# EricPedley/ORB_SLAM3_ROS2

Measured on AMD Instinct MI355X. Metric: frames/sec ORB extract+match @640×480; KF/sec LocalBA (50 KF, 2k pts), higher is better.
Workload: dtype u8; 1 GPU; C2: 640x480, 8-level pyramid, 1000 feat/frame, FAST 20/7, batch=1 per camera stream; ORBextractor::operator() + brute-force Hamming match to the camera's previous frame; step=one frame on each of 16 independent camera streams, parallelism=replicas x1 (no collective); 16 camera streams per GPU, batch 1 each, cameras=16

## Files before the change

### orb_slam3_ros2_amd/csrc/extract.cpp

```cpp
#include "extract.h"

#include <algorithm>
#include <cstdlib>
#include <cstring>
#include <map>
#include <memory>
#include <mutex>
#include <vector>

#include "devbuf.h"
#include "graph_cache.h"
#include "orbhip_kernels.h"
#include "stage.h"

#define HIPOK(x) ORBHIP_HIPOK(" extract", x)

namespace orbhip {
namespace {

struct Plan {
    HostPlan hp;
    DevBuf<ExtractPlan> d_plan;
    DevBuf<CellGeom> d_cells;
    DevBuf<int> d_xofs, d_xalpha, d_yofs, d_ybeta, d_disc, d_cone_tab, d_cone_hi_tab, d_bands, d_flow_dep;
// ... 139 lines not shown
    HIPOK(ws->grow(ws->d_pyr, (size_t)B * P.pyr_bytes));
    HIPOK(ws->grow(ws->d_cand, (size_t)B * P.n_slots_total));
    HIPOK(ws->grow(ws->d_cprim, (size_t)B * P.n_cells_total * kCandPrim));
    HIPOK(ws->grow(ws->d_kscratch, (size_t)B * P.n_slots_total));
    HIPOK(ws->grow(ws->d_nscratch, (size_t)B * P.n_slots_total));
    HIPOK(ws->grow(ws->d_cand_cnt, (size_t)B * P.n_cells_total));
    HIPOK(ws->grow(ws->d_cand_off, (size_t)B * P.n_cells_total));
    HIPOK(ws->grow(ws->d_cand_fill, (size_t)B * kMaxLevels));
    if (pl->hp.flow_nbt) {
        const uint64_t was = ws->gen;
        HIPOK(ws->grow(ws->d_flow, kFlowCtl + (size_t)B * pl->hp.flow_nbt));
        if (ws->gen != was) HIPOK(hipMemset(ws->d_flow.p, 0, ws->d_flow.n * sizeof(int)));
    }
    HIPOK(ws->grow(ws->d_lvl_kp, (size_t)B * P.kp_slots_total));
    HIPOK(ws->grow(ws->d_lvl_cnt, (size_t)B * P.n_levels));
    HIPOK(ws->grow(ws->d_lvl_nlap, (size_t)B * P.n_levels));
    HIPOK(ws->grow(ws->d_err, 4));
    return ORBHIP_OK;
}

static void launch_pyramid(ExtractWorkspace* ws, Plan* pl, FrameBufs& fb, int B, const RunSwitches& sw, bool flow_on,
                           hipStream_t st) {
    const ExtractPlan& P = pl->hp.h;
    StageTimer& tm = *ws->timer;
    static const size_t cone_max = std::getenv("ORBHIP_CONE_MAX_WG")
                                       ? (size_t)std::atol(std::getenv("ORBHIP_CONE_MAX_WG"))
                                       : (size_t)1024;
    const bool cone_path = pl->hp.cone_tiles && !sw.no_cone && (size_t)B * pl->hp.cone_tiles <= cone_max;
    const bool cone_hi = !cone_path && pl->hp.cone_hi_tiles && sw.cone_hi;
    fb.stamp = (cone_path && tm.stage == 1 && tm.dstamp && tm.n < StageTimer::kCap) ? tm.dstamp + tm.n : nullptr;
    if (cone_path) {
        static const int cone_nt = [] {
            const char* e = std::getenv("ORBHIP_CONE_NT");
            const int v = e ? std::atoi(e) : 1024;
            return (v == 256 || v == 512) ? v : 1024;
        }();
        launch_pyr_cone(pl->d_plan.p, pl->hp.cone_tiles, pl->hp.cone_lds, fb, B, pl->d_cone.p, pl->d_cone_tab.p,
                        pl->hp.cone_tab_stride, st, 0, cone_nt, pl->d_xofs.p, pl->d_xalpha.p, pl->d_yofs.p,
                        pl->d_ybeta.p);
    } else if (flow_on) {
        PyrFlow fa{};
        fa.ctl = ws->d_flow.p;
        fa.flags = ws->d_flow.p + kFlowCtl;
        fa.dep = (const int2*)pl->d_flow_dep.p;
        for (int l = 0; l <= kMaxLevels; l++) fa.boff[l] = pl->hp.flow_boff[l];
        fa.B = B;
        fa.nbt = pl->hp.flow_nbt;
        fa.pyr_limit = (int)((int64_t)B * P.pyr_bytes);
        launch_pyr_flow(pl->d_plan.p, fb, pl->d_xofs.p, pl->d_xalpha.p, pl->d_yofs.p, pl->d_ybeta.p, fa, st);
    } else {
        const bool bands = !cone_hi && pl->hp.nbands > 0;
        const int lr = cone_hi ? kConeHiStart + 1 : (bands ? kBandStart + 1 : P.n_levels);
        for (int l = 1; l < lr; l++)
            launch_resize(pl->d_plan.p, P, fb, B, l, pl->d_xofs.p, pl->d_xalpha.p, pl->d_yofs.p, pl->d_ybeta.p,
                          st);
        if (cone_hi)
            launch_pyr_cone(pl->d_plan.p, pl->hp.cone_hi_tiles, pl->hp.cone_hi_lds, fb, B, pl->d_cone_hi.p,
                            pl->d_cone_hi_tab.p, pl->hp.cone_hi_tab_stride, st, kConeHiStart, cone_hi_threads(),
                            pl->d_xofs.p, pl->d_xalpha.p, pl->d_yofs.p, pl->d_ybeta.p);
        if (bands)
            launch_resize_bands(pl->d_plan.p, pl->hp.nbands, fb, B, kBandStart, (const int2*)pl->d_bands.p,
                                pl->d_xofs.p, pl->d_xalpha.p, pl->d_yofs.p, pl->d_ybeta.p, st);
    }
}

static int run_extract(ExtractWorkspace* ws, Plan* pl, const uint8_t* d_imgs, int B, int stride, int64_t fstride,
                       int lap0, int lap1, orbhip_kp* d_kps, uint8_t* d_desc, int cap, int32_t* d_n, int32_t* d_mono,
                       hipStream_t st) {
    const ExtractPlan& P = pl->hp.h;
    (void)hipGetLastError();
    int rc = ensure_batch(ws, pl, B);
    if (rc) return rc;
    const RunSwitches sw = read_run_switches();
    const bool flow_on = sw.flow && pl->hp.flow_nbt > 0 && (int64_t)B * P.pyr_bytes < (1ll << 31);
    GraphKey key;
    key.add(1).add((uint64_t)sw.oct_fast).add((uint64_t)sw.oct_max_dh).add((uint64_t)sw.no_cone)
        .add((uint64_t)sw.cone_hi).add((uint64_t)flow_on).add((uint64_t)sw.pack).add((uint64_t)ws->fast_nt).ptr(pl)
        .ptr(d_imgs).add((uint64_t)B).add((uint64_t)stride).add((uint64_t)fstride).add((uint64_t)lap0)
        .add((uint64_t)lap1).ptr(d_kps).ptr(d_desc).add((uint64_t)cap).ptr(d_n).ptr(d_mono).ptr(st)
        .ptr(ws).add(ws->gen);
    return ws->graphs->run(key, st, ws->timer->stage != 0, [&](hipStream_t st) -> int {
        FrameBufs fb;
        fb.in = d_imgs; fb.in_stride = stride; fb.in_fstride = fstride; fb.pyr = ws->d_pyr.p;
        StageTimer& tm = *ws->timer;
        const StageScope scope(tm);
        tm.begin(1, st);
        launch_pyramid(ws, pl, fb, B, sw, flow_on, st);
        tm.end(1, st);
        tm.begin(2, st);
        CandPack cp;
        cp.prim = ws->d_cprim.p;
        if (sw.pack) {
// ... 191 lines not shown
```

### orb_slam3_ros2_amd/csrc/extract_kernels.hip

```cpp
#include <hip/hip_runtime.h>
#include <cstdlib>
#include <type_traits>

#include "../../include/orbhip.h"
#include "dev_attr.h"
#include "../../include/orbhip_pattern.h"
#include "orbhip_device.h"
#include "orbhip_kernels.h"
#include "orbhip_plan.h"

namespace orbhip {

__constant__ __attribute__((visibility("hidden"))) signed char kPattern[256 * 4] = ORBHIP_BIT_PATTERN_31_INIT;

ORBHIP_TRACE_UNIT(extract)

struct ImgRef {
    const uint8_t* p;
    int pitch;
};

__device__ __forceinline__ ImgRef level_img(const ExtractPlan* __restrict__ P, const FrameBufs& fb, int f, int l) {
    if (l == 0) return ImgRef{fb.in + (int64_t)f * fb.in_fstride, fb.in_stride};
    return ImgRef{fb.pyr + (int64_t)f * P->pyr_bytes + P->lv[l].pyr_off, P->lv[l].pitch};
// ... 279 lines not shown
                        typedef unsigned int u32x4v __attribute__((ext_vector_type(4)));
                        const u32x4v u = {v.x, v.y, v.z, v.w};
                        __builtin_amdgcn_raw_buffer_store_b128(u, prs, obase + (dyb + r) * pitch + c, 0, 16);
                    }
                    wave_lds_only();
                }
            }
            asm volatile("s_waitcnt vmcnt(0)" ::: "memory");
            __syncthreads();
            if (tid == 0)
                __hip_atomic_store((ex_gint*)(fl + a.boff[l] + b), gen + 1, __ATOMIC_RELAXED,
                                   __HIP_MEMORY_SCOPE_AGENT);
            if (tr_k < 32) { TR_PHASE(7, 2 * tr_k + 1) }
            tr_k++;
        }
    }
    TR_END(7)
    if (tid == 0 && atomicAdd(ctl + kFlowQ, 1) == (int)gridDim.x - 1) {
        for (int i = 0; i <= kFlowQ; i++)
            __hip_atomic_store((ex_gint*)(ctl + i), 0, __ATOMIC_RELAXED, __HIP_MEMORY_SCOPE_AGENT);
        __hip_atomic_store((ex_gint*)(ctl + kFlowQ + 1), gen + 1, __ATOMIC_RELAXED, __HIP_MEMORY_SCOPE_AGENT);
    }
}

__device__ __forceinline__ int small_div(int i, float inv_d) { return (int)(((float)i + 0.5f) * inv_d); }

__device__ __forceinline__ void wait_vm_all() { asm volatile("s_waitcnt vmcnt(0)" ::: "memory"); }
__device__ __forceinline__ void lds_only_barrier() {
    asm volatile("s_waitcnt lgkmcnt(0)" ::: "memory");
    __builtin_amdgcn_s_barrier();
    asm volatile("" ::: "memory");
}

__device__ __forceinline__ void pyr_cone_body(const ExtractPlan* __restrict__ P, const FrameBufs& fb,
                                              const ConeRect* __restrict__ rects, const int* __restrict__ ctab,
                                              int tab_stride, uint8_t* __restrict__ cone, int tile, int f, int s0) {
    TR_BEGIN()
    const int L = P->n_levels, tid = threadIdx.x, nt = blockDim.x;
    const ConeRect* R = rects + (size_t)tile * kMaxLevels;
    static_assert(sizeof(ConeRect) == 16 && kMaxLevels * 4 <= 64 && (kMaxLevels & (kMaxLevels - 1)) == 0, "4 dwords per level");
    const uint32_t rdw = ((const uint32_t*)R)[threadIdx.x & (4 * kMaxLevels - 1)];
    auto rect = [&](int l) -> ConeRect {
        const uint32_t d0 = (uint32_t)__builtin_amdgcn_readlane((int)rdw, 4 * l),
                       d1 = (uint32_t)__builtin_amdgcn_readlane((int)rdw, 4 * l + 1),
                       d2 = (uint32_t)__builtin_amdgcn_readlane((int)rdw, 4 * l + 2),
                       d3 = (uint32_t)__builtin_amdgcn_readlane((int)rdw, 4 * l + 3);
        return ConeRect{(int16_t)(d0 & 0xFFFF), (int16_t)(d0 >> 16), (int16_t)(d1 & 0xFFFF), (int16_t)(d1 >> 16),
                        (int16_t)(d2 & 0xFFFF), (int16_t)(d2 >> 16), (int16_t)(d3 & 0xFFFF), (int16_t)(d3 >> 16)};
    };
    int boff[kMaxLevels], toff[kMaxLevels];
    int tot = 0;
    const ConeRect Rs0 = rect(s0);
    const int P0 = (Rs0.nx1 - Rs0.nx0 + 6) & ~3;
    for (int l = s0; l < L; l++) {
        const ConeRect r = rect(l);
        boff[l] = tot;
        tot += ((l == s0 ? P0 : (r.nx1 - r.nx0)) * (r.ny1 - r.ny0) + 15) & ~15;
    }
    int sh0 = 0;
    int* tab = (int*)(cone + tot);
    int ttot = 0;
    for (int l = s0 + 1; l < L; l++) {
        toff[l] = ttot;
        const ConeRect r = rect(l);
        ttot += 2 * (r.nx1 - r.nx0) + 3 * (r.ny1 - r.ny0);
    }
    const int* gt = ctab + (size_t)tile * tab_stride;
    auto tab_at = [&](int i) -> int { return gt[i]; };
    TR_PHASE(0, 20)
    {
        const ImgRef in0 = level_img(P, fb, f, s0);
        const ConeRect r = Rs0;
        const int nw = r.nx1 - r.nx0, nh = r.ny1 - r.ny0;
        const uint8_t* src0 = in0.p + (int64_t)r.ny0 * in0.pitch + r.nx0;
        const bool dw = ((in0.pitch & 3) == 0) && ((((uintptr_t)in0.p) & 3) == 0);
        if (dw) sh0 = (int)(((uintptr_t)src0) & 3);
        const int nwd = dw ? (nw + sh0 + 3) >> 2 : 0;
        const int tot0 = dw ? nwd * nh : nw * nh;
        const float inv_n = 1.0f / (float)(dw ? nwd : nw);
        uint8_t* lv0 = cone + boff[s0];
        if (dw && tot0 <= 1024 && ttot <= 2 * 1024 && nt == 1024) {
            const uint32_t* s4 = (const uint32_t*)(src0 - sh0);
            const int p4 = in0.pitch >> 2;
            int tv[2];
#pragma unroll
            for (int u = 0; u < 2; u++) tv[u] = gt[min(tid + 1024 * u, ttot - 1)];
            const int i = min(tid, tot0 - 1);
            const int y = small_div(i, inv_n), x = i - y * nwd;
            const uint32_t v = s4[(int64_t)y * p4 + x];
#pragma unroll
            for (int u = 0; u < 2; u++)
                if (tid + 1024 * u < ttot) tab[tid + 1024 * u] = tv[u];
            if (tid < tot0) ((uint32_t*)lv0)[y * (P0 >> 2) + x] = v;
            TR_PHASE(0, 21)
        } else if (dw) {
            const uint32_t* s4 = (const uint32_t*)(src0 - sh0);
            const int p4 = in0.pitch >> 2;
            constexpr int U = 8;
            for (int i0 = tid; i0 < ttot; i0 += U * nt) {
                int v[U];
#pragma unroll
                for (int u = 0; u < U; u++) v[u] = tab_at(min(i0 + u * nt, ttot - 1));
#pragma unroll
                for (int u = 0; u < U; u++)
                    if (i0 + u * nt < ttot) tab[i0 + u * nt] = v[u];
            }
            for (int i0 = tid; i0 < tot0; i0 += U * nt) {
                uint32_t v[U];
                int o[U];
#pragma unroll
                for (int u = 0; u < U; u++) {
                    const int i = min(i0 + u * nt, tot0 - 1);
                    const int y = small_div(i, inv_n), x = i - y * nwd;
                    v[u] = s4[(int64_t)y * p4 + x];
                    o[u] = y * (P0 >> 2) + x;
                }
#pragma unroll
                for (int u = 0; u < U; u++)
                    if (i0 + u * nt < tot0) ((uint32_t*)lv0)[o[u]] = v[u];
            }
        } else {
            for (int i = tid; i < ttot; i += nt) tab[i] = tab_at(i);
            for (int i = tid; i < tot0; i += nt) {
                const int y = small_div(i, inv_n), x = i - y * nw;
                lv0[y * P0 + x] = src0[(int64_t)y * in0.pitch + x];
            }
        }
    }
    __syncthreads();
    TR_PHASE(0, 0)
    for (int l = s0 + 1; l < L; l++) {
        const LevelGeom& D = P->lv[l];
        const ConeRect r = rect(l), rp = rect(l - 1);
        const int nw = r.nx1 - r.nx0, nh = r.ny1 - r.ny0, nwp = l == s0 + 1 ? P0 : rp.nx1 - rp.nx0;
        const int* t = tab + toff[l];
        const uint8_t* src = cone + boff[l - 1] + (l == s0 + 1 ? sh0 : 0);
        uint8_t* dst = fb.pyr + (int64_t)f * P->pyr_bytes + D.pyr_off;
        const float inv_nw = 1.0f / (float)nw;
        const bool noclamp = D.rz_noclamp != 0;
        for (int i = tid; i < nw * nh; i += nt) {
            const int yy = small_div(i, inv_nw), xx = i - yy * nw;
            const int x = r.nx0 + xx, y = r.ny0 + yy;
            const int sx = t[xx] - rp.nx0;
            const uint8_t* S0 = src + (t[2 * nw + 3 * yy] - rp.ny0) * nwp;
            const uint8_t* S1 = src + (t[2 * nw + 3 * yy + 1] - rp.ny0) * nwp;
            int h0, h1;
            if (x < D.xmax) {
                const int aa = t[nw + xx];
                const int a0 = (int)(short)(aa & 0xFFFF), a1 = (int)(short)(aa >> 16);
                h0 = S0[sx] * a0 + S0[sx + 1] * a1;
                h1 = S1[sx] * a0 + S1[sx + 1] * a1;
            } else {
                h0 = S0[sx] * 2048;
                h1 = S1[sx] * 2048;
            }
            const int bb = t[2 * nw + 3 * yy + 2];
            const int b0 = (int)(short)(bb & 0xFFFF), b1 = (int)(short)(bb >> 16);
            int v;
            if (x < D.vend && noclamp) {
                v = ((__mul24(h0 >> 4, b0) >> 16) + (__mul24(h1 >> 4, b1) >> 16) + 2) >> 2;
            } else if (x < D.vend) {
                int s0 = min(max(h0 >> 4, -32768), 32767);
                int s1 = min(max(h1 >> 4, -32768), 32767);
                int tt = ((s0 * b0) >> 16) + ((s1 * b1) >> 16);
                tt = min(max(tt, -32768), 32767);
                v = (tt + 2) >> 2;
            } else {
                v = (h0 * b0 + h1 * b1 + (1 << 21)) >> 22;
            }
            const uint8_t u = (uint8_t)(v < 0 ? 0 : (v > 255 ? 255 : v));
            cone[boff[l] + i] = u;
            if (x >= r.ox0 && x < r.ox1 && y >= r.oy0 && y < r.oy1) dst[(int64_t)y * D.pitch + x] = u;
        }
        lds_only_barrier();
        TR_PHASE(0, l)
    }
    TR_END(0)
}

__global__ __launch_bounds__(1024) void k_pyr_cone(const ExtractPlan* __restrict__ P, FrameBufs fb,
                                                   const ConeRect* __restrict__ rects, const int* __restrict__ ctab,
                                                   int tab_stride, int xrun, int s0) {
    extern __shared__ __attribute__((aligned(16))) uint8_t cone[];
    if (fb.stamp && threadIdx.x == 0) atomicMin(fb.stamp, (unsigned long long)__builtin_amdgcn_s_memrealtime());
    const int X = gridDim.x, lg = xcd_runs(blockIdx.x + X * blockIdx.y, X * gridDim.y, xrun < 0 ? X : xrun);
    pyr_cone_body(P, fb, rects, ctab, tab_stride, cone, lg % X, lg / X, s0);
    if (fb.stamp) {
        __syncthreads();
        if (threadIdx.x == 0) atomicMax(fb.stamp + kStampStride, (unsigned long long)__builtin_amdgcn_s_memrealtime());
    }
}

constexpr int kWinMax = 80;
#ifndef ORBHIP_OCT_W0_MAIN
#define ORBHIP_OCT_W0_MAIN 1
#endif
#ifndef ORBHIP_OCT_BLK_FINAL
#define ORBHIP_OCT_BLK_FINAL 1
#endif
typedef _Float16 h2 __attribute__((ext_vector_type(2)));
typedef unsigned short u16x2 __attribute__((ext_vector_type(2)));
constexpr uint32_t kPwBias = 0x64006400u;

__device__ __forceinline__ h2 as_h2(uint32_t u) { return __builtin_bit_cast(h2, u); }
__device__ __forceinline__ h2 hmin(h2 a, h2 b) { return __builtin_elementwise_minimum(a, b); }
__device__ __forceinline__ h2 hmax(h2 a, h2 b) { return __builtin_elementwise_maximum(a, b); }

template <int P>
struct Circle {
    static constexpr int o[17] = {6 * P + 3, 6 * P + 4, 5 * P + 5, 4 * P + 6, 3 * P + 6, 2 * P + 6,
                                  P + 5,     4,         3,         2,         P + 1,     2 * P,
                                  3 * P,     4 * P,     5 * P + 1, 6 * P + 2, 3 * P + 3};
};

template <int WR>
struct FastShape {
    static constexpr bool full = WR >= kWinMax;
    static constexpr int wmax = full ? kWinMax : 45;
    static constexpr int pwp = ((wmax + 3 + 3) / 4) * 4;
// ... 1592 lines not shown
        o.size = (float)G.patch_size;
        o.angle = angle;
        o.response = (float)(kp.srl & 0xFF);
        o.octave = l;
        out_kps[(int64_t)f * cap + idx] = o;
    }
}

static int xcd_run_for(int B) {
    static const int env = getenv("ORBHIP_XCD_RUN") ? atoi(getenv("ORBHIP_XCD_RUN")) : -2;
    return env >= -1 ? env : (B >= 8 ? -1 : (B > 1 ? 16 : 8));
}

void launch_resize(const ExtractPlan* dP, const ExtractPlan& hP, const FrameBufs& fb, int B, int l,
                   const int* xofs, const int* xalpha, const int* yofs, const int* ybeta, hipStream_t st) {
    const LevelGeom& D = hP.lv[l];
    dim3 blk(64, 4, 1);
    dim3 grd((D.h + 4 * kRzRows - 1) / (4 * kRzRows), (D.w + 255) / 256, B);
    ORBHIP_LAUNCH(k_resize, grd, blk, 0, st, dP, fb, l, xofs, xalpha, yofs, ybeta);
}

void launch_pyr_flow(const ExtractPlan* dP, const FrameBufs& fb, const int* xofs, const int* xalpha, const int* yofs,
                     const int* ybeta, const PyrFlow& a, hipStream_t st) {
    const int ntask = a.B * a.boff[kMaxLevels];
    const int grid = std::max(kFlowQ, std::min((ntask + kFlowChunk - 1) / kFlowChunk, 1024));
    ORBHIP_LAUNCH(k_pyr_flow, dim3(grid), dim3(256), 0, st, dP, fb, xofs, xalpha, yofs, ybeta, a);
}

void launch_resize_bands(const ExtractPlan* dP, int nbands, const FrameBufs& fb, int B, int s0, const int2* rows,
                         const int* xofs, const int* xalpha, const int* yofs, const int* ybeta, hipStream_t st) {
    ORBHIP_LAUNCH(k_resize_bands, dim3(nbands, B), dim3(256), 0, st, dP, fb, s0, rows, xofs, xalpha, yofs, ybeta);
}

void launch_pyr_cone(const ExtractPlan* dP, int ntiles, size_t lds, const FrameBufs& fb, int B, const ConeRect* rects,
                     const int* ctab, int tab_stride, hipStream_t st, int s0, int nthreads, const int* xofs,
                     const int* xalpha, const int* yofs, const int* ybeta) {
    static LdsAttrOnce attr;
    (void)attr.ensure((const void*)k_pyr_cone, 64 * 1024);
    (void)xofs; (void)xalpha; (void)yofs; (void)ybeta;
    ORBHIP_LAUNCH(k_pyr_cone, dim3(ntiles, B), dim3(nthreads), lds, st, dP, fb, rects, ctab, tab_stride,
                  xcd_run_for(B), s0);
}

void launch_fast(const ExtractPlan* dP, const ExtractPlan& hP, const CellGeom* cells, const FrameBufs& fb, int B,
                 uint32_t* cand, int* cand_cnt, int* err, hipStream_t st, int nt_hint, CandPack cp) {
    const int ncell = B * hP.n_cells_total;
    const int nt = hP.fast_nt ? hP.fast_nt
                              : (nt_hint ? nt_hint
                                         : (ncell <= 512 ? 1024 : (ncell <= 1024 ? 512 : (ncell <= 32768 ? 256 : 128))));
    dim3 grd(hP.n_cells_total, B, 1);
    const int xr = xcd_run_for(B);
    const bool compact = hP.fast_win_rows <= 50 && hP.fast_win_cols <= 45;
#define ORBHIP_FAST_LAUNCH(NTV, WRV) \
    ORBHIP_LAUNCH((k_fast_cells<NTV, WRV>), grd, dim3(NTV), 0, st, dP, cells, fb, cand, cand_cnt, err, xr, cp)
    if (nt == 1024 && compact)
        ORBHIP_FAST_LAUNCH(1024, 50);
    else if (nt == 1024)
        ORBHIP_FAST_LAUNCH(1024, kWinMax);
    else if (nt == 512 && compact)
        ORBHIP_FAST_LAUNCH(512, 50);
    else if (nt == 512)
        ORBHIP_FAST_LAUNCH(512, kWinMax);
    else if (nt == 128 && compact)
        ORBHIP_FAST_LAUNCH(128, 50);
    else if (nt == 128)
        ORBHIP_FAST_LAUNCH(128, kWinMax);
    else if (compact)
        ORBHIP_FAST_LAUNCH(256, 50);
    else
        ORBHIP_FAST_LAUNCH(256, kWinMax);
#undef ORBHIP_FAST_LAUNCH
}

void launch_octree(const ExtractPlan* dP, const ExtractPlan& hP, const CellGeom* cells, const uint16_t* otab,
// ... 39 lines not shown
```

### orb_slam3_ros2_amd/csrc/extract_plan.cpp

```cpp
#include "extract_plan.h"

#include <algorithm>
#include <cfloat>
#include <cstdio>
#include <cstdlib>

namespace orbhip {

static int round_even_d(double v) { return (int)std::nearbyint(v); }
static int floor_f(float v) { int i = (int)v; return i - (i > v); }
static short sat_s16(int v) { return (short)std::min(std::max(v, -32768), 32767); }

OrbTables build_orb_tables(const orbhip_orb_params& prm) {
    OrbTables t;
    const int L = prm.n_levels;
    const double sf = (double)prm.scale_factor;
    t.scale.assign(L, 1.f);
    t.inv_scale.assign(L, 1.f);
    for (int i = 1; i < L; i++) t.scale[i] = (float)(t.scale[i - 1] * sf);
    for (int i = 0; i < L; i++) t.inv_scale[i] = 1.0f / t.scale[i];
    t.feat.assign(L, 0);
    const float factor = (float)(1.0f / sf);
    float nd = prm.n_features * (1 - factor) / (1 - (float)std::pow((double)factor, (double)L));
    int sum = 0;
// ... 60 lines not shown
        *a0 = pl.xofs[U.xtab_off + nx0];
        *a1 = pl.xofs[U.xtab_off + nx1 - 1] + ((nx1 - 1) < U.xmax ? 1 : 0) + 1;
        auto clampr = [&](int r) { return r < 0 ? 0 : (r < G.h ? r : G.h - 1); };
        *b0 = clampr(pl.yofs[U.ytab_off + ny0]);
        *b1 = clampr(pl.yofs[U.ytab_off + ny1 - 1] + 1) + 1;
    };
    for (int ti = 0; ti < nty; ti++)
        for (int tj = 0; tj < ntx; tj++) {
            ConeRect* R = &rects[((size_t)ti * ntx + tj) * kMaxLevels];
            int nx0 = 0, nx1 = 0, ny0 = 0, ny1 = 0;
            for (int l = L - 1; l > s0; l--) {
                const LevelGeom& G = P.lv[l];
                const int ox0 = (int)((int64_t)tj * G.w / ntx), ox1 = (int)((int64_t)(tj + 1) * G.w / ntx);
                const int oy0 = (int)((int64_t)ti * G.h / nty), oy1 = (int)((int64_t)(ti + 1) * G.h / nty);
                int a0 = ox0, a1 = ox1, b0 = oy0, b1 = oy1;
                if (l < L - 1 && nx1 > nx0 && ny1 > ny0) {
                    int lo, hi, r0, r1;
                    source_of(l + 1, nx0, nx1, ny0, ny1, &lo, &hi, &r0, &r1);
                    a0 = std::min(a0, lo); a1 = std::max(a1, hi);
                    b0 = std::min(b0, r0); b1 = std::max(b1, r1);
                    if (ox1 <= ox0 || oy1 <= oy0) { a0 = lo; a1 = hi; b0 = r0; b1 = r1; }
                }
                R[l] = ConeRect{(int16_t)a0, (int16_t)a1, (int16_t)b0, (int16_t)b1,
                                (int16_t)ox0, (int16_t)ox1, (int16_t)oy0, (int16_t)oy1};
                nx0 = a0; nx1 = a1; ny0 = b0; ny1 = b1;
            }
            {
                int lo, hi, r0, r1;
                source_of(s0 + 1, nx0, nx1, ny0, ny1, &lo, &hi, &r0, &r1);
                R[s0] = ConeRect{(int16_t)lo, (int16_t)hi, (int16_t)r0, (int16_t)r1, 0, 0, 0, 0};
            }
            size_t tot = 0, ttot = 0;
            for (int l = s0; l < L; l++) {
                const size_t wl = l == s0 ? (size_t)((R[s0].nx1 - R[s0].nx0 + 6) & ~3) : (size_t)(R[l].nx1 - R[l].nx0);
                tot += (wl * (R[l].ny1 - R[l].ny0) + 15) & ~size_t(15);
            }
            for (int l = s0 + 1; l < L; l++)
                ttot += 4 * (2 * (size_t)(R[l].nx1 - R[l].nx0) + 3 * (size_t)(R[l].ny1 - R[l].ny0));
            lds_max = std::max(lds_max, tot + ttot);
        }
    tab_stride = 0;
    for (int t = 0; t < ntx * nty; t++) {
        size_t tt = 0;
        for (int l = s0 + 1; l < L; l++) {
            const ConeRect& r = rects[(size_t)t * kMaxLevels + l];
            tt += 2 * (size_t)(r.nx1 - r.nx0) + 3 * (size_t)(r.ny1 - r.ny0);
        }
        tab_stride = std::max(tab_stride, tt);
    }
    ctab.assign((size_t)ntx * nty * tab_stride, 0);
    for (int t = 0; t < ntx * nty; t++) {
        int* o = ctab.data() + (size_t)t * tab_stride;
        for (int l = s0 + 1; l < L; l++) {
            const LevelGeom& D = P.lv[l];
            const LevelGeom& S = P.lv[l - 1];
            const ConeRect r = rects[(size_t)t * kMaxLevels + l];
            const int nw = r.nx1 - r.nx0, nh = r.ny1 - r.ny0;
            for (int i = 0; i < nw; i++) {
                o[i] = pl.xofs[D.xtab_off + r.nx0 + i];
                o[nw + i] = pl.xalpha[D.xtab_off + r.nx0 + i];
            }
            auto clampr = [&](int v) { return v < 0 ? 0 : (v < S.h ? v : S.h - 1); };
            for (int j = 0; j < nh; j++) {
                const int sy = pl.yofs[D.ytab_off + r.ny0 + j];
                o[2 * nw + 3 * j] = clampr(sy);
                o[2 * nw + 3 * j + 1] = clampr(sy + 1);
                o[2 * nw + 3 * j + 2] = pl.ybeta[D.ytab_off + r.ny0 + j];
// ... 269 lines not shown
```

### orb_slam3_ros2_amd/csrc/orbhip_kernels.h

```cpp
#pragma once
#include <hip/hip_ext.h>
#include <hip/hip_runtime.h>
#include <stddef.h>
#include <stdint.h>

#include "../../include/orbhip.h"
#include "orbhip_plan.h"

namespace orbhip {

struct FrameBufs {
    const uint8_t* in;
    int in_stride;
    int64_t in_fstride;
    uint8_t* pyr;
    unsigned long long* stamp = nullptr;
};
constexpr int kStampStride = 8192;

struct StageTimer;
inline thread_local StageTimer* g_stage_timer = nullptr;
struct StageTimer {
    int stage = 0;
    int n = 0;
    static constexpr int kCap = 8192;
    hipEvent_t ev[2 * kCap];
    bool created = false;
    bool used = false;
    unsigned long long* dstamp = nullptr;
    void begin(int s, hipStream_t) {
        if (s == stage && n < kCap) { used = false; g_stage_timer = this; }
    }
    void end(int s, hipStream_t) {
        if (s == stage && g_stage_timer == this) { g_stage_timer = nullptr; if (used) n++; }
    }
};
struct StageScope {
    StageTimer& t;
    explicit StageScope(StageTimer& tm) : t(tm) {}
    ~StageScope() {
        if (g_stage_timer == &t) g_stage_timer = nullptr;
    }
};

#define ORBHIP_LAUNCH(kern, grid, block, shm, st, ...)                                                          \
    do {                                                                                                      \
        ::orbhip::StageTimer* t_ = ::orbhip::g_stage_timer;                                                   \
        if (t_) {                                                                                             \
            hipExtLaunchKernelGGL(kern, grid, block, (uint32_t)(shm), st, t_->used ? nullptr : t_->ev[2 * t_->n], \
                                  t_->ev[2 * t_->n + 1], 0u, __VA_ARGS__);                                    \
            t_->used = true;                                                                                  \
        } else {                                                                                              \
            hipLaunchKernelGGL(kern, grid, block, shm, st, __VA_ARGS__);                                      \
        }                                                                                                     \
    } while (0)

void launch_pyr_cone(const ExtractPlan* dP, int ntiles, size_t lds, const FrameBufs& fb, int B, const ConeRect* rects,
                     const int* ctab, int tab_stride, hipStream_t st, int s0 = 0, int nthreads = 1024,
                     const int* xofs = nullptr, const int* xalpha = nullptr, const int* yofs = nullptr,
                     const int* ybeta = nullptr);
void launch_resize_bands(const ExtractPlan* dP, int nbands, const FrameBufs& fb, int B, int s0, const int2* rows,
                         const int* xofs, const int* xalpha, const int* yofs, const int* ybeta, hipStream_t st);
void launch_resize(const ExtractPlan* dP, const ExtractPlan& hP, const FrameBufs& fb, int B, int l,
                   const int* xofs, const int* xalpha, const int* yofs, const int* ybeta, hipStream_t st);
constexpr int kFlowQ = 8;
constexpr int kFlowChunk = 1;
constexpr int kFlowCtl = 16;
struct PyrFlow {
    int* ctl;
    int* flags;
    const int2* dep;
    int boff[kMaxLevels + 1];
    int B;
    int nbt;
    int pyr_limit;
};
void launch_pyr_flow(const ExtractPlan* dP, const FrameBufs& fb, const int* xofs, const int* xalpha, const int* yofs,
                     const int* ybeta, const PyrFlow& a, hipStream_t st);
struct CandPack {
    int* fill = nullptr;
    int* off = nullptr;
    uint32_t* prim = nullptr;
};
constexpr int kCandPrim = 16;
void launch_fast(const ExtractPlan* dP, const ExtractPlan& hP, const CellGeom* cells, const FrameBufs& fb, int B,
                 uint32_t* cand, int* cand_cnt, int* err, hipStream_t st, int nt_hint = 0, CandPack cp = {});
bool octree_set_lds_limit(size_t bytes);
void launch_octree(const ExtractPlan* dP, const ExtractPlan& hP, const CellGeom* cells, const uint16_t* otab,
                   const uint32_t* cand, const uint32_t* cprim,
                   const int* cand_cnt, const int* cand_off, uint32_t* kscratch, uint16_t* nscratch, LevelKp* lvl_kp,
                   int* lvl_cnt, int* lvl_nlap, const OctreeCfg& cfg, int* err, int B, hipStream_t st,
                   unsigned long long* stamp = nullptr);
void launch_desc(const ExtractPlan* dP, const ExtractPlan& hP, const FrameBufs& fb, const LevelKp* lvl_kp,
// ... 135 lines not shown
```

### orb_slam3_ros2_amd/csrc/orbhip_plan.h

```cpp
#pragma once
#include <stddef.h>
#include <stdint.h>

#if !defined(__HIPCC__) && !defined(__host__)
#define __host__
#define __device__
#endif

namespace orbhip {

constexpr int kMaxLevels = 16;
constexpr int kPatchR = 21;
constexpr int kPatchW = 2 * kPatchR + 1;
constexpr int kDiscMax = 1024;

struct LevelGeom {
    int w, h, pitch;
    int64_t pyr_off;
    float scale;
    int n_feat;
    int min_bx, max_bx, min_by, max_by;
    int n_cols, n_rows, w_cell, h_cell;
    int cell_base, n_cells;
    int slot_base, n_slots;
// ... 5 lines not shown
    int patch_size;
    int xtab_off, ytab_off, xmax, vend;
};

struct CellGeom {
    int16_t level, pad;
    int16_t x0, y0;
    int16_t wc, hc;
    int32_t slot_off;
};

constexpr int kClistCap = 2048;

struct ExtractPlan {
    int w, h, n_levels;
    int n_cells_total, n_slots_total;
    int kp_slots_total;
    int64_t pyr_bytes;
    int ini_th, min_th;
    int n_disc;
    int blurk[7];
    int max_cells_level;
    int clist_cap;
    int fast_nt;
    int fast_win_rows, fast_win_cols;
    LevelGeom lv[kMaxLevels];
};

struct ConeRect {
    int16_t nx0, nx1, ny0, ny1;
    int16_t ox0, ox1, oy0, oy1;
};

__host__ __device__ inline uint32_t pack_cand(int x, int y, int score) {
    return (uint32_t)x | ((uint32_t)y << 12) | ((uint32_t)score << 24);
}
__host__ __device__ inline int cand_x(uint32_t c) { return (int)(c & 0xFFF); }
__host__ __device__ inline int cand_y(uint32_t c) { return (int)((c >> 12) & 0xFFF); }
__host__ __device__ inline int cand_s(uint32_t c) { return (int)(c >> 24); }

struct LevelKp {
    int16_t x, y;
    uint32_t srl;
};

struct OctreeCfg {
    int node_cap;
    int sort_cap;
    int key_cap;
    int lap0, lap1;
    int fast;
    int max_dh;
};

inline size_t octree_lds_bytes(const ExtractPlan& hP, const OctreeCfg& cfg) {
    size_t off = 0;
    auto carve = [&](size_t bytes) { off += (bytes + 15) & ~size_t(15); };
    const size_t NC = cfg.node_cap;
    carve(64 * 4);
    for (int b = 0; b < 2; b++) { carve(NC * 8); carve(NC * 4); carve(NC * 4); carve(NC * 4); }
    carve(NC * 16); carve(NC * 16); carve(NC * 8);
    carve(NC * 4); carve(NC * 4); carve(NC * 4); carve(NC * 4);
    carve((size_t)cfg.sort_cap * 8);
    carve((size_t)cfg.sort_cap * 8);
    carve((size_t)(hP.max_cells_level + 1) * 4);
    carve((size_t)(hP.max_cells_level + 1) * 4);
// ... 7 lines not shown
```

Before: 44380 frames/s.

## Vectorize pyramid cone resize into 4-pixel dword groups with packed sdot2

Rewrites the pyramid cone kernel so each thread produces four output pixels at once. Source bytes are read as dwords, shuffled with perm/alignbyte and combined with sdot2, and results are written as packed dword stores. Per-level cone buffers in LDS get a 4-byte-aligned pitch, and per-level geometry (pitch, offset, xmax, vend) is passed by value as a kernel argument instead of read from the device plan. The default block size drops from 1024 to 512 threads, with the level-0 copy path generalized to use two pixels per thread. This adds a scalar fallback for edge groups and slightly more LDS, and the packed path has to reproduce the scalar rounding exactly.

```diff
diff --git a/orb_slam3_ros2_amd/csrc/extract.cpp b/orb_slam3_ros2_amd/csrc/extract.cpp
--- a/orb_slam3_ros2_amd/csrc/extract.cpp
+++ b/orb_slam3_ros2_amd/csrc/extract.cpp
@@ -195,12 +195,11 @@
     if (cone_path) {
         static const int cone_nt = [] {
             const char* e = std::getenv("ORBHIP_CONE_NT");
-            const int v = e ? std::atoi(e) : 1024;
-            return (v == 256 || v == 512) ? v : 1024;
+            const int v = e ? std::atoi(e) : 512;
+            return (v == 256 || v == 1024) ? v : 512;
         }();
-        launch_pyr_cone(pl->d_plan.p, pl->hp.cone_tiles, pl->hp.cone_lds, fb, B, pl->d_cone.p, pl->d_cone_tab.p,
-                        pl->hp.cone_tab_stride, st, 0, cone_nt, pl->d_xofs.p, pl->d_xalpha.p, pl->d_yofs.p,
-                        pl->d_ybeta.p);
+        launch_pyr_cone(pl->d_plan.p, P, pl->hp.cone_tiles, pl->hp.cone_lds, fb, B, pl->d_cone.p, pl->d_cone_tab.p,
+                        pl->hp.cone_tab_stride, st, 0, cone_nt);
     } else if (flow_on) {
         PyrFlow fa{};
         fa.ctl = ws->d_flow.p;
@@ -218,9 +217,8 @@
             launch_resize(pl->d_plan.p, P, fb, B, l, pl->d_xofs.p, pl->d_xalpha.p, pl->d_yofs.p, pl->d_ybeta.p,
                           st);
         if (cone_hi)
-            launch_pyr_cone(pl->d_plan.p, pl->hp.cone_hi_tiles, pl->hp.cone_hi_lds, fb, B, pl->d_cone_hi.p,
-                            pl->d_cone_hi_tab.p, pl->hp.cone_hi_tab_stride, st, kConeHiStart, cone_hi_threads(),
-                            pl->d_xofs.p, pl->d_xalpha.p, pl->d_yofs.p, pl->d_ybeta.p);
+            launch_pyr_cone(pl->d_plan.p, P, pl->hp.cone_hi_tiles, pl->hp.cone_hi_lds, fb, B, pl->d_cone_hi.p,
+                            pl->d_cone_hi_tab.p, pl->hp.cone_hi_tab_stride, st, kConeHiStart, cone_hi_threads());
         if (bands)
             launch_resize_bands(pl->d_plan.p, pl->hp.nbands, fb, B, kBandStart, (const int2*)pl->d_bands.p,
                                 pl->d_xofs.p, pl->d_xalpha.p, pl->d_yofs.p, pl->d_ybeta.p, st);
diff --git a/orb_slam3_ros2_amd/csrc/extract_kernels.hip b/orb_slam3_ros2_amd/csrc/extract_kernels.hip
--- a/orb_slam3_ros2_amd/csrc/extract_kernels.hip
+++ b/orb_slam3_ros2_amd/csrc/extract_kernels.hip
@@ -335,12 +335,52 @@
     asm volatile("" ::: "memory");
 }
 
+__device__ __forceinline__ int cone_px(const int* t, int nw, int xx, int yy, const uint8_t* src, int spitch,
+                                       int snx0, int sny0, int x, int xmax, int vend, bool noclamp) {
+    const int sx = t[xx] - snx0;
+    const uint8_t* S0 = src + (t[2 * nw + 3 * yy] - sny0) * spitch;
+    const uint8_t* S1 = src + (t[2 * nw + 3 * yy + 1] - sny0) * spitch;
+    int h0, h1;
+    if (x < xmax) {
+        const int aa = t[nw + xx];
+        const int a0 = (int)(short)(aa & 0xFFFF), a1 = (int)(short)(aa >> 16);
+        h0 = S0[sx] * a0 + S0[sx + 1] * a1;
+        h1 = S1[sx] * a0 + S1[sx + 1] * a1;
+    } else {
+        h0 = S0[sx] * 2048;
+        h1 = S1[sx] * 2048;
+    }
+    const int bb = t[2 * nw + 3 * yy + 2];
+    const int b0 = (int)(short)(bb & 0xFFFF), b1 = (int)(short)(bb >> 16);
+    int v;
+    if (x < vend && noclamp) {
+        v = ((__mul24(h0 >> 4, b0) >> 16) + (__mul24(h1 >> 4, b1) >> 16) + 2) >> 2;
+    } else if (x < vend) {
+        int s0 = min(max(h0 >> 4, -32768), 32767);
+        int s1 = min(max(h1 >> 4, -32768), 32767);
+        int tt = ((s0 * b0) >> 16) + ((s1 * b1) >> 16);
+        tt = min(max(tt, -32768), 32767);
+        v = (tt + 2) >> 2;
+    } else {
+        v = (h0 * b0 + h1 * b1 + (1 << 21)) >> 22;
+    }
+    return v < 0 ? 0 : (v > 255 ? 255 : v);
+}
+
+__device__ __forceinline__ float small_div_rcp(int d) { return __builtin_amdgcn_rcpf((float)d); }
+
 __device__ __forceinline__ void pyr_cone_body(const ExtractPlan* __restrict__ P, const FrameBufs& fb,
                                               const ConeRect* __restrict__ rects, const int* __restrict__ ctab,
-                                              int tab_stride, uint8_t* __restrict__ cone, int tile, int f, int s0) {
+                                              int tab_stride, uint8_t* __restrict__ cone, int tile, int f, int s0,
+                                              const ConeGeom& geom) {
     TR_BEGIN()
     const int L = P->n_levels, tid = threadIdx.x, nt = blockDim.x;
+    const int64_t pyr_bytes = P->pyr_bytes;
+    uint8_t* pyr_f = fb.pyr + (int64_t)f * pyr_bytes;
+    asm volatile("" : "+s"(pyr_f));
     const ConeRect* R = rects + (size_t)tile * kMaxLevels;
+    const int gdw = geom.v[threadIdx.x & (4 * kMaxLevels - 1)];
+    auto geo = [&](int l, int k) -> int { return __builtin_amdgcn_readlane(gdw, 4 * l + k); };
     static_assert(sizeof(ConeRect) == 16 && kMaxLevels * 4 <= 64 && (kMaxLevels & (kMaxLevels - 1)) == 0, "4 dwords per level");
     const uint32_t rdw = ((const uint32_t*)R)[threadIdx.x & (4 * kMaxLevels - 1)];
     auto rect = [&](int l) -> ConeRect {
@@ -351,23 +391,17 @@
         return ConeRect{(int16_t)(d0 & 0xFFFF), (int16_t)(d0 >> 16), (int16_t)(d1 & 0xFFFF), (int16_t)(d1 >> 16),
                         (int16_t)(d2 & 0xFFFF), (int16_t)(d2 >> 16), (int16_t)(d3 & 0xFFFF), (int16_t)(d3 >> 16)};
     };
-    int boff[kMaxLevels], toff[kMaxLevels];
-    int tot = 0;
     const ConeRect Rs0 = rect(s0);
     const int P0 = (Rs0.nx1 - Rs0.nx0 + 6) & ~3;
-    for (int l = s0; l < L; l++) {
+    const int cb0 = (P0 * (Rs0.ny1 - Rs0.ny0) + 15) & ~15;
+    int tot = cb0, ttot = 0;
+    for (int l = s0 + 1; l < L; l++) {
         const ConeRect r = rect(l);
-        boff[l] = tot;
-        tot += ((l == s0 ? P0 : (r.nx1 - r.nx0)) * (r.ny1 - r.ny0) + 15) & ~15;
+        tot += (cone_pitch(r.nx0, r.nx1 - r.nx0) * (r.ny1 - r.ny0) + 15) & ~15;
+        ttot += 2 * (r.nx1 - r.nx0) + 3 * (r.ny1 - r.ny0);
     }
     int sh0 = 0;
     int* tab = (int*)(cone + tot);
-    int ttot = 0;
-    for (int l = s0 + 1; l < L; l++) {
-        toff[l] = ttot;
-        const ConeRect r = rect(l);
-        ttot += 2 * (r.nx1 - r.nx0) + 3 * (r.ny1 - r.ny0);
-    }
     const int* gt = ctab + (size_t)tile * tab_stride;
     auto tab_at = [&](int i) -> int { return gt[i]; };
     TR_PHASE(0, 20)
@@ -380,21 +414,28 @@
         if (dw) sh0 = (int)(((uintptr_t)src0) & 3);
         const int nwd = dw ? (nw + sh0 + 3) >> 2 : 0;
         const int tot0 = dw ? nwd * nh : nw * nh;
-        const float inv_n = 1.0f / (float)(dw ? nwd : nw);
-        uint8_t* lv0 = cone + boff[s0];
-        if (dw && tot0 <= 1024 && ttot <= 2 * 1024 && nt == 1024) {
+        const float inv_n = small_div_rcp(dw ? nwd : nw);
+        uint8_t* lv0 = cone;
+        if (dw && tot0 <= 2 * nt && ttot <= 4 * nt) {
             const uint32_t* s4 = (const uint32_t*)(src0 - sh0);
             const int p4 = in0.pitch >> 2;
-            int tv[2];
-#pragma unroll
-            for (int u = 0; u < 2; u++) tv[u] = gt[min(tid + 1024 * u, ttot - 1)];
-            const int i = min(tid, tot0 - 1);
-            const int y = small_div(i, inv_n), x = i - y * nwd;
-            const uint32_t v = s4[(int64_t)y * p4 + x];
+            int tv[4], o[2];
+            uint32_t v[2];
+#pragma unroll
+            for (int u = 0; u < 4; u++) tv[u] = gt[min(tid + nt * u, ttot - 1)];
+#pragma unroll
+            for (int u = 0; u < 2; u++) {
+                const int i = min(tid + nt * u, tot0 - 1);
+                const int y = small_div(i, inv_n), x = i - y * nwd;
+                v[u] = s4[(int64_t)y * p4 + x];
+                o[u] = y * (P0 >> 2) + x;
+            }
+#pragma unroll
+            for (int u = 0; u < 4; u++)
+                if (tid + nt * u < ttot) tab[tid + nt * u] = tv[u];
 #pragma unroll
             for (int u = 0; u < 2; u++)
-                if (tid + 1024 * u < ttot) tab[tid + 1024 * u] = tv[u];
-            if (tid < tot0) ((uint32_t*)lv0)[y * (P0 >> 2) + x] = v;
+                if (tid + nt * u < tot0) ((uint32_t*)lv0)[o[u]] = v[u];
             TR_PHASE(0, 21)
         } else if (dw) {
             const uint32_t* s4 = (const uint32_t*)(src0 - sh0);
@@ -432,62 +473,122 @@
     }
     __syncthreads();
     TR_PHASE(0, 0)
+    typedef short short2v __attribute__((ext_vector_type(2)));
+    int cbp = 0, cb = cb0, tb = 0;
+    int lpp = sh0, Pp = P0;
     for (int l = s0 + 1; l < L; l++) {
-        const LevelGeom& D = P->lv[l];
         const ConeRect r = rect(l), rp = rect(l - 1);
-        const int nw = r.nx1 - r.nx0, nh = r.ny1 - r.ny0, nwp = l == s0 + 1 ? P0 : rp.nx1 - rp.nx0;
-        const int* t = tab + toff[l];
-        const uint8_t* src = cone + boff[l - 1] + (l == s0 + 1 ? sh0 : 0);
-        uint8_t* dst = fb.pyr + (int64_t)f * P->pyr_bytes + D.pyr_off;
-        const float inv_nw = 1.0f / (float)nw;
-        const bool noclamp = D.rz_noclamp != 0;
-        for (int i = tid; i < nw * nh; i += nt) {
-            const int yy = small_div(i, inv_nw), xx = i - yy * nw;
+        const int nw = r.nx1 - r.nx0, nh = r.ny1 - r.ny0;
+        const int lp = r.nx0 & 3, Pl = cone_pitch(r.nx0, nw), gpr = Pl >> 2;
+        const int g0 = geo(l, 0), pitch = g0 & 0x7FFFFFFF, xmax = geo(l, 2), vend = geo(l, 3);
+        const bool noclamp = g0 < 0;
+        const int* t = tab + tb;
+        const uint8_t* srcb = cone + cbp;
+        const uint8_t* src = srcb + lpp;
+        uint8_t* const out = cone + cb;
+        uint8_t* const dst = pyr_f + ((int64_t)geo(l, 1) << 6);
+        const float inv_gpr = small_div_rcp(gpr);
+        const int snx0 = rp.nx0, sny0 = rp.ny0;
+        const int ox0 = r.ox0, ox1 = r.ox1, oy0 = r.oy0, oy1 = r.oy1;
+        for (int g = tid; g < gpr * nh; g += nt) {
+            const int yy = small_div(g, inv_gpr), gx = g - yy * gpr;
+            const int xx = 4 * gx - lp;
             const int x = r.nx0 + xx, y = r.ny0 + yy;
-            const int sx = t[xx] - rp.nx0;
-            const uint8_t* S0 = src + (t[2 * nw + 3 * yy] - rp.ny0) * nwp;
-            const uint8_t* S1 = src + (t[2 * nw + 3 * yy + 1] - rp.ny0) * nwp;
-            int h0, h1;
-            if (x < D.xmax) {
-                const int aa = t[nw + xx];
-                const int a0 = (int)(short)(aa & 0xFFFF), a1 = (int)(short)(aa >> 16);
-                h0 = S0[sx] * a0 + S0[sx + 1] * a1;
-                h1 = S1[sx] * a0 + S1[sx + 1] * a1;
+            const int k0 = max(0, -xx), k1 = min(4, nw - xx);
+            int xo[4], xa[4];
+#pragma unroll
+            for (int k = 0; k < 4; k++) xo[k] = t[xx + k];
+#pragma unroll
+            for (int k = 0; k < 4; k++) xa[k] = t[nw + xx + k];
+            const int r0 = t[2 * nw + 3 * yy], r1 = t[2 * nw + 3 * yy + 1], bb = t[2 * nw + 3 * yy + 2];
+#pragma unroll
+            for (int k = 1; k < 4; k++) {
+                xo[k] = k >= k1 ? xo[k - 1] : xo[k];
+                xa[k] = k >= k1 ? xa[k - 1] : xa[k];
+            }
+#pragma unroll
+            for (int k = 2; k >= 0; k--) {
+                xo[k] = k < k0 ? xo[k + 1] : xo[k];
+                xa[k] = k < k0 ? xa[k + 1] : xa[k];
+            }
+            const int xf = x + k0, xl = x + k1 - 1;
+            const bool inx = xl < xmax, vecy = xl < vend && noclamp;
+            const int mn = min(min(xo[0], xo[1]), min(xo[2], xo[3]));
+            const int mx = max(max(xo[0], xo[1]), max(xo[2], xo[3]));
+            const bool packed_ok = (inx || xf >= xmax) && (vecy || xf >= vend) && mx - mn <= 6;
+            const bool rowown = y >= oy0 && y < oy1;
+            uint8_t* const d = dst + (int64_t)y * pitch + x;
+            if (packed_ok) {
+                const int sb = mn - snx0 + lpp, sh = sb & 3;
+                const uint32_t* A = (const uint32_t*)(srcb + (r0 - sny0) * Pp + (sb & ~3));
+                const uint32_t* B = (const uint32_t*)(srcb + (r1 - sny0) * Pp + (sb & ~3));
+                const uint32_t a0 = A[0], a1 = A[1], a2 = A[2], c0 = B[0], c1 = B[1], c2 = B[2];
+                const uint32_t wa0 = __builtin_amdgcn_alignbyte(a1, a0, sh), wa1 = __builtin_amdgcn_alignbyte(a2, a1, sh);
+                const uint32_t wc0 = __builtin_amdgcn_alignbyte(c1, c0, sh), wc1 = __builtin_amdgcn_alignbyte(c2, c1, sh);
+                const uint32_t sel0 = inx ? 0x0C010C00u : 0x0C0C0C00u, selm = inx ? 0x00010001u : 1u;
+                const int b0 = (int)(short)(bb & 0xFFFF), b1 = (int)(short)(bb >> 16);
+                int h0[4], h1[4];
+#pragma unroll
+                for (int k = 0; k < 4; k++) {
+                    const uint32_t sel = sel0 + __umul24((uint32_t)(xo[k] - mn), selm);
+                    const short2v av = __builtin_bit_cast(short2v, inx ? xa[k] : 2048);
+                    h0[k] = __builtin_amdgcn_sdot2(
+                        __builtin_bit_cast(short2v, __builtin_amdgcn_perm(wa1, wa0, sel)), av, 0, false);
+                    h1[k] = __builtin_amdgcn_sdot2(
+                        __builtin_bit_cast(short2v, __builtin_amdgcn_perm(wc1, wc0, sel)), av, 0, false);
+                }
+                uint32_t pk = 0;
+                if (vecy) {
+#pragma unroll
+                    for (int k = 0; k < 4; k++) {
+                        const int v = ((__mul24(h0[k] >> 4, b0) >> 16) + (__mul24(h1[k] >> 4, b1) >> 16) + 2) >> 2;
+                        pk |= (uint32_t)min(max(v, 0), 255) << (8 * k);
+                    }
+                } else {
+#pragma unroll
+                    for (int k = 0; k < 4; k++) {
+                        const int v = (h0[k] * b0 + h1[k] * b1 + (1 << 21)) >> 22;
+                        pk |= (uint32_t)min(max(v, 0), 255) << (8 * k);
+                    }
+                }
+                *(uint32_t*)(out + yy * Pl + 4 * gx) = pk;
+                if (rowown) {
+                    if (x >= ox0 && x + 3 < ox1) {
+                        *(uint32_t*)d = pk;
+                    } else {
+#pragma unroll
+                        for (int k = 0; k < 4; k++)
+                            if (x + k >= ox0 && x + k < ox1) d[k] = (uint8_t)(pk >> (8 * k));
+                    }
+                }
             } else {
-                h0 = S0[sx] * 2048;
-                h1 = S1[sx] * 2048;
-            }
-            const int bb = t[2 * nw + 3 * yy + 2];
-            const int b0 = (int)(short)(bb & 0xFFFF), b1 = (int)(short)(bb >> 16);
-            int v;
-            if (x < D.vend && noclamp) {
-                v = ((__mul24(h0 >> 4, b0) >> 16) + (__mul24(h1 >> 4, b1) >> 16) + 2) >> 2;
-            } else if (x < D.vend) {
-                int s0 = min(max(h0 >> 4, -32768), 32767);
-                int s1 = min(max(h1 >> 4, -32768), 32767);
-                int tt = ((s0 * b0) >> 16) + ((s1 * b1) >> 16);
-                tt = min(max(tt, -32768), 32767);
-                v = (tt + 2) >> 2;
-            } else {
-                v = (h0 * b0 + h1 * b1 + (1 << 21)) >> 22;
-            }
-            const uint8_t u = (uint8_t)(v < 0 ? 0 : (v > 255 ? 255 : v));
-            cone[boff[l] + i] = u;
-            if (x >= r.ox0 && x < r.ox1 && y >= r.oy0 && y < r.oy1) dst[(int64_t)y * D.pitch + x] = u;
+#pragma unroll 1
+                for (int k = k0; k < k1; k++) {
+                    const uint8_t u =
+                        (uint8_t)cone_px(t, nw, xx + k, yy, src, Pp, snx0, sny0, x + k, xmax, vend, noclamp);
+                    out[yy * Pl + 4 * gx + k] = u;
+                    if (rowown && x + k >= ox0 && x + k < ox1) d[k] = u;
+                }
+            }
         }
         lds_only_barrier();
         TR_PHASE(0, l)
+        cbp = cb;
+        cb += (Pl * nh + 15) & ~15;
+        tb += 2 * nw + 3 * nh;
+        lpp = lp;
+        Pp = Pl;
     }
     TR_END(0)
 }
 
 __global__ __launch_bounds__(1024) void k_pyr_cone(const ExtractPlan* __restrict__ P, FrameBufs fb,
                                                    const ConeRect* __restrict__ rects, const int* __restrict__ ctab,
-                                                   int tab_stride, int xrun, int s0) {
+                                                   int tab_stride, int xrun, int s0, ConeGeom geom) {
     extern __shared__ __attribute__((aligned(16))) uint8_t cone[];
     if (fb.stamp && threadIdx.x == 0) atomicMin(fb.stamp, (unsigned long long)__builtin_amdgcn_s_memrealtime());
     const int X = gridDim.x, lg = xcd_runs(blockIdx.x + X * blockIdx.y, X * gridDim.y, xrun < 0 ? X : xrun);
-    pyr_cone_body(P, fb, rects, ctab, tab_stride, cone, lg % X, lg / X, s0);
+    pyr_cone_body(P, fb, rects, ctab, tab_stride, cone, lg % X, lg / X, s0, geom);
     if (fb.stamp) {
         __syncthreads();
         if (threadIdx.x == 0) atomicMax(fb.stamp + kStampStride, (unsigned long long)__builtin_amdgcn_s_memrealtime());
@@ -2146,14 +2247,20 @@
     ORBHIP_LAUNCH(k_resize_bands, dim3(nbands, B), dim3(256), 0, st, dP, fb, s0, rows, xofs, xalpha, yofs, ybeta);
 }
 
-void launch_pyr_cone(const ExtractPlan* dP, int ntiles, size_t lds, const FrameBufs& fb, int B, const ConeRect* rects,
-                     const int* ctab, int tab_stride, hipStream_t st, int s0, int nthreads, const int* xofs,
-                     const int* xalpha, const int* yofs, const int* ybeta) {
+void launch_pyr_cone(const ExtractPlan* dP, const ExtractPlan& hP, int ntiles, size_t lds, const FrameBufs& fb, int B,
+                     const ConeRect* rects, const int* ctab, int tab_stride, hipStream_t st, int s0, int nthreads) {
     static LdsAttrOnce attr;
     (void)attr.ensure((const void*)k_pyr_cone, 64 * 1024);
-    (void)xofs; (void)xalpha; (void)yofs; (void)ybeta;
+    ConeGeom geom{};
+    for (int l = 1; l < hP.n_levels; l++) {
+        const LevelGeom& G = hP.lv[l];
+        geom.v[4 * l] = G.pitch | (G.rz_noclamp ? (int)0x80000000u : 0);
+        geom.v[4 * l + 1] = (int)(G.pyr_off >> 6);
+        geom.v[4 * l + 2] = G.xmax;
+        geom.v[4 * l + 3] = G.vend;
+    }
     ORBHIP_LAUNCH(k_pyr_cone, dim3(ntiles, B), dim3(nthreads), lds, st, dP, fb, rects, ctab, tab_stride,
-                  xcd_run_for(B), s0);
+                  xcd_run_for(B), s0, geom);
 }
 
 void launch_fast(const ExtractPlan* dP, const ExtractPlan& hP, const CellGeom* cells, const FrameBufs& fb, int B,
diff --git a/orb_slam3_ros2_amd/csrc/extract_plan.cpp b/orb_slam3_ros2_amd/csrc/extract_plan.cpp
--- a/orb_slam3_ros2_amd/csrc/extract_plan.cpp
+++ b/orb_slam3_ros2_amd/csrc/extract_plan.cpp
@@ -116,7 +116,8 @@
             }
             size_t tot = 0, ttot = 0;
             for (int l = s0; l < L; l++) {
-                const size_t wl = l == s0 ? (size_t)((R[s0].nx1 - R[s0].nx0 + 6) & ~3) : (size_t)(R[l].nx1 - R[l].nx0);
+                const size_t wl = l == s0 ? (size_t)((R[s0].nx1 - R[s0].nx0 + 6) & ~3)
+                                          : (size_t)cone_pitch(R[l].nx0, R[l].nx1 - R[l].nx0);
                 tot += (wl * (R[l].ny1 - R[l].ny0) + 15) & ~size_t(15);
             }
             for (int l = s0 + 1; l < L; l++)
diff --git a/orb_slam3_ros2_amd/csrc/orbhip_kernels.h b/orb_slam3_ros2_amd/csrc/orbhip_kernels.h
--- a/orb_slam3_ros2_amd/csrc/orbhip_kernels.h
+++ b/orb_slam3_ros2_amd/csrc/orbhip_kernels.h
@@ -55,10 +55,8 @@
         }                                                                                                     \
     } while (0)
 
-void launch_pyr_cone(const ExtractPlan* dP, int ntiles, size_t lds, const FrameBufs& fb, int B, const ConeRect* rects,
-                     const int* ctab, int tab_stride, hipStream_t st, int s0 = 0, int nthreads = 1024,
-                     const int* xofs = nullptr, const int* xalpha = nullptr, const int* yofs = nullptr,
-                     const int* ybeta = nullptr);
+void launch_pyr_cone(const ExtractPlan* dP, const ExtractPlan& hP, int ntiles, size_t lds, const FrameBufs& fb, int B,
+                     const ConeRect* rects, const int* ctab, int tab_stride, hipStream_t st, int s0, int nthreads);
 void launch_resize_bands(const ExtractPlan* dP, int nbands, const FrameBufs& fb, int B, int s0, const int2* rows,
                          const int* xofs, const int* xalpha, const int* yofs, const int* ybeta, hipStream_t st);
 void launch_resize(const ExtractPlan* dP, const ExtractPlan& hP, const FrameBufs& fb, int B, int l,
diff --git a/orb_slam3_ros2_amd/csrc/orbhip_plan.h b/orb_slam3_ros2_amd/csrc/orbhip_plan.h
--- a/orb_slam3_ros2_amd/csrc/orbhip_plan.h
+++ b/orb_slam3_ros2_amd/csrc/orbhip_plan.h
@@ -61,6 +61,12 @@
     int16_t ox0, ox1, oy0, oy1;
 };
 
+__host__ __device__ inline int cone_pitch(int nx0, int nw) { return ((nx0 & 3) + nw + 3) & ~3; }
+
+struct ConeGeom {
+    int v[4 * kMaxLevels];
+};
+
 __host__ __device__ inline uint32_t pack_cand(int x, int y, int score) {
     return (uint32_t)x | ((uint32_t)y << 12) | ((uint32_t)score << 24);
 }
```

Measured after the change: 43880 frames/s. 1.1% lower.
